# manasakani/Accelerated-Kinetic-Monte-Carlo-simulations-of-atomistically-resolved-resistive-memory-arrays

Hardware: AMD Instinct MI355X
Metric: cg_iterations_per_sec (higher is better)
Workload: dtype f64; 1 GPU; synthetic_40nm_crossbar(tiles=8,fill=0.52,lines=2,seed=40,bwmin); rows=1597080, nnz=41834706, sites=1635480, partition=1-D block rows x 1, transport=single, solver=jacobi-pcg fixed 1411 iterations, halo_cols_rank0=0, neighbours_rank0=1

## Files before the change

accelerated-kinetic-monte-carlo-simulations-of-atomistically-resolved-resistive-memory-arrays_amd/csrc/kmcf_internal.hpp:

```cpp
#pragma once
#include <hip/hip_runtime.h>

#include <condition_variable>
#include <cstdarg>
#include <cstdint>
#include <cstdio>
#include <algorithm>
#include <cstdlib>
#include <mutex>
#include <type_traits>
#include <vector>

#include "kmcfield.h"
#include "kmcf_knobs.hpp"

void kmcf_set_error(const char *fmt, ...);

#define KMCF_HIP(call)                                                                       \
    do {                                                                                     \
        hipError_t e_ = (call);                                                              \
        if (e_ != hipSuccess) {                                                              \
            kmcf_set_error("%s:%d: %s -> %s", __FILE__, __LINE__, #call, hipGetErrorString(e_)); \
            return KMCF_ERR_HIP;                                                             \
        }                                                                                    \
// ... 188 lines not shown
    int spmv_grid_coded = 0;
    bool sell_ok = false;
    bool sell_dirty = true;
    std::vector<int> h_sell_cuts;
    bool sell_ident = false;
    bool sell_nt = false;
    int sell_lw = 10, sell_nq = 0;
    int n_sell_tiles = 0, sell_grid = 0;
    int64_t n_sell_wcols = 0, n_sell_entries = 0;
    int4 *d_sell_tile = nullptr;
    int2 *d_sell_wave = nullptr;
    int *d_sell_lrow = nullptr;
    int *d_sell_wcol = nullptr;
    unsigned short *d_sell = nullptr;
    int *d_sell_pos = nullptr;
    double *d_sellv = nullptr;
    bool sellv_dirty = true;
    int sellv_grid = 0;
    int n_chunks = 0;
    int *d_chunk_row = nullptr;
    std::vector<int> h_row_ptr;
};

struct kmcf_kstate {
    kmcf_comm *comm = nullptr;
    kmcf_matrix *K = nullptr;
    int N = 0, N_left = 0, N_right = 0, N_interface = 0;
    std::vector<int> h_row_ptr, h_col;
    std::vector<int> h_left_row_ptr, h_left_col, h_right_row_ptr, h_right_col;
    int *d_left_row_ptr = nullptr, *d_left_col = nullptr;
// ... 37 lines not shown
    KMCF_PATH_STREAM,
    KMCF_PATH_WINDOW,
    KMCF_PATH_WCODE,
    KMCF_PATH_SELL,
    KMCF_PATH_SELLV,
};

inline kmcf_spmv_path kmcf_interior_path(const kmcf_matrix *m)
{
    if (m->spmv_kind == 1) return KMCF_PATH_STREAM;
    if (m->spmv_kind != 2) return KMCF_PATH_VEC;
    if (m->coded && m->sell_ok && m->dict_n <= 3) return KMCF_PATH_SELL;
    if (!m->coded && m->sell_ok && m->sell_ident && m->sellv_grid > 0) return KMCF_PATH_SELLV;
    return m->coded ? KMCF_PATH_WCODE : KMCF_PATH_WINDOW;
}

inline int kmcf_interior_grid(const kmcf_matrix *m)
{
    switch (kmcf_interior_path(m)) {
        case KMCF_PATH_WCODE: return m->spmv_grid_coded;
        case KMCF_PATH_SELL: return m->sell_grid;
        case KMCF_PATH_SELLV: return m->sellv_grid;
        default: return m->spmv_grid;
    }
}

constexpr int KMCF_SELL_NQ[] = {8, 13, 16};

template <class F>
int kmcf_sell_instance(const kmcf_matrix *m, F &&f)
// ... 157 lines not shown
```

accelerated-kinetic-monte-carlo-simulations-of-atomistically-resolved-resistive-memory-arrays_amd/csrc/kmcf_knobs.hpp:

```cpp
#pragma once
#include <cstdlib>
#include <string>

enum kmcf_knob_id {
    KNOB_BRICK, KNOB_SPMV_KIND, KNOB_SPMV_CODED, KNOB_SPMV_SELL, KNOB_SPMV_SELLV, KNOB_SPMV_SELL_ROWS,
    KNOB_SPMV_SELL_SORT, KNOB_SPMV_NT, KNOB_SELL_NT, KNOB_LONG_ROW, KNOB_CB_SCALED, KNOB_SUB_DENSE, KNOB_SUB_STRIP,
    KNOB_EVENTS_PERSISTENT, KNOB_EVENTS_FULLSCAN, KNOB_EVENTS_PARTITIONED, KNOB_EV_TREL, KNOB_CG_VARIANT,
    KNOB_CG_RESIDENT, KNOB_CGR_TPB, KNOB_CGR_G1, KNOB_CGR_DELAY, KNOB_CGR_RDELAY, KNOB_CGR_ADAPT, KNOB_CGR_TIMEOUT_MS,
    KNOB_CGR_CLASSIC_TILES, KNOB_TRANSPORT, KNOB_P2P_WINDOW_MB, KNOB_P2P_TIMEOUT_MS, KNOB_P2P_DIRECT, KNOB_P2P_AR,
    KNOB_FORCE_COMM, KNOB_LOOPBACK_TIMEOUT_S, KNOB_DEVICE_SHARE, KNOB_ENTER_ALWAYS, KNOB_TRACE, KNOB_COUNT
};

enum kmcf_knob_scope { KNOB_SCOPE_NONE, KNOB_COMM, KNOB_CONNECT, KNOB_PROCESS };

enum kmcf_knob_kind { KNOB_SPEC_NONE, KNOB_ENUM, KNOB_INT, KNOB_F64, KNOB_FLAG };
struct kmcf_knob_spec {
    kmcf_knob_kind kind;
    const char *words;
    double lo, hi;
};
constexpr kmcf_knob_spec kv_enum(const char *words) { return {KNOB_ENUM, words, 0, 0}; }
constexpr kmcf_knob_spec kv_int(double lo, double hi) { return {KNOB_INT, nullptr, lo, hi}; }
constexpr kmcf_knob_spec kv_f64(double lo, double hi) { return {KNOB_F64, nullptr, lo, hi}; }
constexpr kmcf_knob_spec kv_flag() { return {KNOB_FLAG, "0|1", 0, 0}; }
// ... 12 lines not shown
    {KNOB_SPMV_KIND, "KMCF_SPMV_KIND", "window, else stream, else vec", "0 vec / 1 stream / 2 window", "SpMV kernel family (forced: the window plan is not judged)",
     KNOB_COMM, false, kv_enum("0|1|2")},
    {KNOB_SPMV_CODED, "KMCF_SPMV_CODED", "1", "0 / 1", "0: f64 values streamed even where they could be coded",
     KNOB_COMM, false, kv_enum("0|1")},
    {KNOB_SPMV_SELL, "KMCF_SPMV_SELL", "1", "0 / 1", "0: the coded window kernel instead of the row-per-lane kernel",
     KNOB_COMM, false, kv_enum("0|1")},
    {KNOB_SPMV_SELLV, "KMCF_SPMV_SELLV", "1", "0 / 1", "0: f64 matrices on the window kernel instead of the row-per-lane one",
     KNOB_COMM, false, kv_enum("0|1")},
    {KNOB_SPMV_SELL_ROWS, "KMCF_SPMV_SELL_ROWS", "by size: 64 … 256", "64 … 256 (multiples of 64)", "rows per row-per-lane tile",
     KNOB_COMM, false, kv_enum("64|128|192|256")},
    {KNOB_SPMV_SELL_SORT, "KMCF_SPMV_SELL_SORT", "1", "0 / 1", "0: the rows of a tile are not sorted into the internal row order",
     KNOB_COMM, false, kv_enum("0|1")},
    {KNOB_SPMV_NT, "KMCF_SPMV_NT", "matrices beyond the caches", "0 / 1", "nontemporal matrix loads in the f64-value SpMV kernels",
     KNOB_COMM, false, kv_enum("0|1")},
    {KNOB_SELL_NT, "KMCF_SELL_NT", "beyond the Infinity Cache", "0 / 1", "nontemporal loads of the coded entry stream",
     KNOB_COMM, false, kv_enum("0|1")},
    {KNOB_LONG_ROW, "KMCF_LONG_ROW", "384", "entries; <= 0: none", "rows longer than this go to the long-row kernel",
     KNOB_COMM, false, kv_int(-1000000000, 1000000000)},
    {KNOB_CB_SCALED, "KMCF_CB_SCALED", "0", "0 / 1", "1: the CB-edge solve in the literal scaled form (a group: one more halo exchange)",
     KNOB_COMM, true, kv_enum("0|1")},
    {KNOB_SUB_DENSE, "KMCF_SUB_DENSE", "dense from a quarter full", "0 bitmap / 1 dense / 2 jagged",
     "tunnel block as bitmap / dense symmetric tiles / jagged tiles (one rank); all ranks of a group must agree",
     KNOB_COMM, true, kv_enum("0|1|2")},
    {KNOB_SUB_STRIP, "KMCF_SUB_STRIP", "16", ">= 1", "tunnel-block tiles per strip",
     KNOB_COMM, true, kv_int(1, 1000000)},
    {KNOB_EVENTS_PERSISTENT, "KMCF_EVENTS_PERSISTENT", "1", "0 / 1", "0: three launches per event instead of one persistent block per batch",
     KNOB_COMM, true, kv_enum("0|1")},
    {KNOB_EVENTS_FULLSCAN, "KMCF_EVENTS_FULLSCAN", "unset", "set", "the reference-style zero-out pass over the event list",
     KNOB_COMM, false, kv_flag()},
    {KNOB_EVENTS_PARTITIONED, "KMCF_EVENTS_PARTITIONED", "unset", "set", "the reference's partitioned multi-rank event step instead of the replicated one",
// ... 78 lines not shown
```

accelerated-kinetic-monte-carlo-simulations-of-atomistically-resolved-resistive-memory-arrays_amd/csrc/kmcf_matrix.hip:

```cpp
#include <algorithm>
#include <cstring>

#include "kmcf_internal.hpp"

namespace {

template <typename T>
int dev_upload(T **d, const std::vector<T> &h)
{
    size_t bytes = std::max<size_t>(h.size(), 1) * sizeof(T);
    KMCF_HIP(hipMalloc(reinterpret_cast<void **>(d), bytes));
    if (!h.empty()) KMCF_HIP(hipMemcpy(*d, h.data(), h.size() * sizeof(T), hipMemcpyHostToDevice));
    return KMCF_OK;
}

template <typename T>
int dev_alloc(T **d, size_t n)
{
    KMCF_HIP(hipMalloc(reinterpret_cast<void **>(d), std::max<size_t>(n, 1) * sizeof(T)));
    KMCF_HIP(hipMemset(*d, 0, std::max<size_t>(n, 1) * sizeof(T)));
    return KMCF_OK;
}

}
// ... 413 lines not shown
    KMCF_CHECK(m && info, KMCF_ERR_ARG, "kmcf_matrix_info: null argument");
    info->matrix_size = m->matrix_size;
    info->rows_this_rank = m->n_loc;
    info->nnz = m->nnz;
    info->number_of_neighbours = m->number_of_neighbours;
    info->halo_cols = m->n_halo;
    info->send_rows = m->n_send;
    info->boundary_rows = m->n_boundary_rows;
    info->spmv_kind = m->spmv_kind;
    const kmcf_spmv_path path = kmcf_interior_path(m);
    const bool sell = path == KMCF_PATH_SELL || path == KMCF_PATH_SELLV;
    const bool window = path == KMCF_PATH_WINDOW || path == KMCF_PATH_WCODE;
    info->spmv_coded = path == KMCF_PATH_SELL ? 2 : path == KMCF_PATH_WCODE ? 1 : 0;
    info->spmv_tiles = sell ? m->n_sell_tiles : window ? m->n_tiles : 0;
    info->spmv_window_cols = sell ? m->n_sell_wcols : window ? m->n_wcols : 0;
    info->spmv_stream_entries = sell ? m->n_sell_entries : path == KMCF_PATH_WCODE ? (int64_t)m->h_row_ptr[m->n_short] : 0;
    return KMCF_OK;
}

extern "C" int kmcf_matrix_neighbour(const kmcf_matrix *m, int k, int *neighbour_rank, int *nnz_block,
                                     int *ncols, int *h_cols, int *nrows, int *h_rows)
{
    KMCF_CHECK(m && k >= 0 && k < m->number_of_neighbours, KMCF_ERR_ARG, "kmcf_matrix_neighbour: k=%d out of range", k);
    if (neighbour_rank) *neighbour_rank = m->neighbours[k];
    if (nnz_block) *nnz_block = m->nnz_per_neighbour[k];
    if (ncols) *ncols = (int)m->cols_per_neighbour[k].size();
    if (nrows) *nrows = (int)m->rows_per_neighbour[k].size();
    if (h_cols) memcpy(h_cols, m->cols_per_neighbour[k].data(), m->cols_per_neighbour[k].size() * sizeof(int));
    if (h_rows) memcpy(h_rows, m->rows_per_neighbour[k].data(), m->rows_per_neighbour[k].size() * sizeof(int));
    return KMCF_OK;
}
// ... 43 lines not shown
```

accelerated-kinetic-monte-carlo-simulations-of-atomistically-resolved-resistive-memory-arrays_amd/csrc/kmcf_spmv.hip:

```cpp
#include <algorithm>
#include <cstdio>
#include <cstdlib>
#include <cstring>

#include <climits>

#include "kmcf_p2p_dev.hpp"

namespace {

__device__ __forceinline__ double wave_sum_width(double v, int width)
{
#pragma unroll
    for (int off = 32; off >= 1; off >>= 1)
        if (off < width) v += __shfl_xor(v, off, 64);
    return v;
}

__device__ __forceinline__ double block_sum_256(double v, double *lds4)
{
    v = kmcf_wave_sum64(v);
    const int lane = threadIdx.x & 63, w = threadIdx.x >> 6;
    if (lane == 0) lds4[w] = v;
    __syncthreads();
// ... 266 lines not shown
    }
}

typedef unsigned int sell_pair __attribute__((ext_vector_type(2)));
#define KMCF_SELL_LD(p) stream_load<NT>(p)
#define KMCF_SELL_LD2(p) (*(p))

template <int WQ>
struct sell_regs {
    double xr[WQ];
    double xrow, xown, dg;
    int row, nq, wn;
    bool valid;
};

template <int NQ, int LW, int ND, bool DOT, bool SKIP_BOUNDARY, bool IDENT, bool NT = false>
__global__ __launch_bounds__(KMCF_BLOCK) void spmv_sell_kernel(
    int n_tiles, const int4 *__restrict__ tile4, const int2 *__restrict__ swave, const int *__restrict__ lrow,
    const int *__restrict__ wcol, const sell_pair *__restrict__ stream, const double *__restrict__ x, double *__restrict__ y,
    const unsigned char *__restrict__ is_boundary, double *__restrict__ part, const kmcf_scalars *__restrict__ S,
    int check_done, const double *__restrict__ dict, const double *__restrict__ diagv)
{
    constexpr int W = 1 << LW, WQ = W / KMCF_BLOCK - 1, BUF = ND * W;
    typedef sell_regs<WQ> regs_t;
    __shared__ double xs[2 * BUF];
    if (check_done && S->done) return;
    const int tid = threadIdx.x;
    const int lane = tid & 63;
    const int wv = __builtin_amdgcn_readfirstlane(tid >> 6);
    double dv[ND];
#pragma unroll
    for (int c = 0; c < ND; ++c) dv[c] = dict[c];
    const int xcd = blockIdx.x & 7, bi = blockIdx.x >> 3, nb8 = gridDim.x >> 3;
    const int Cx = (n_tiles + 7) >> 3;
    const int gmax = min(Cx, n_tiles - xcd * Cx);
    const int nt = gmax > bi ? (gmax - bi + nb8 - 1) / nb8 : 0;
    double dot = 0.0;
    if (nt > 0) {
// ... 18 lines not shown
            } else {
                t.valid = lr >= 0;
                t.row = d.x + (t.valid ? lr : 0);
            }
            t.xrow = x[t.row];
            t.xown = IDENT ? t.xrow : x[d.x + min(tid, d.y - 1)];
            t.dg = KMCF_SELL_LD2(diagv + t.row);
            if (SKIP_BOUNDARY) t.valid = t.valid && is_boundary[t.row] == 0;
            t.nq = sw.y;
            t.wn = d.w;
        };
        int4 d1 = tile4[KMCF_TILE_OF(1)], d2 = tile4[KMCF_TILE_OF(2)];
        int2 s1 = swave[KMCF_TILE_OF(1) * 4 + wv], s2 = swave[KMCF_TILE_OF(2) * 4 + wv];
        int wca[WQ], wcb[WQ], lra = 0, lrb = 0;
        regs_t ta, tb;
        sell_pair pk[NQ];
        {
            const int4 d0 = tile4[c_first];
            const int2 s0 = swave[c_first * 4 + wv];
            load_b(c_first, d0, wca, lra);
            load_b_pinned(KMCF_TILE_OF(1), d1, wcb, lrb);
            __builtin_amdgcn_sched_barrier(0);
            load_c(d0, s0, wca, lra, ta);
            const sell_pair *sp = stream + s0.x + lane;
            const int last = max(s0.y - 1, 0);
#pragma unroll
            for (int q = 0; q < NQ; ++q) pk[q] = KMCF_SELL_LD(sp + min(q, last) * 64);
        }
        auto body = [&](int k, regs_t &cur, regs_t &nxt, double *xb, int (&wu)[WQ], int &lu, int (&wl)[WQ], int &ll) {
#pragma unroll
            for (int c = 0; c < ND; ++c) xb[c * W + tid] = dv[c] * cur.xown;
#pragma unroll
            for (int q = 0; q < WQ; ++q) {
                const int slot = q * KMCF_BLOCK + tid;
                const double v = slot < cur.wn ? cur.xr[q] : 0.0;
#pragma unroll
                for (int c = 0; c < ND; ++c) xb[c * W + KMCF_BLOCK + slot] = dv[c] * v;
            }
            load_b(KMCF_TILE_OF(k + 2), d2, wl, ll);
            __builtin_amdgcn_sched_barrier(0);
            load_c(d1, s1, wu, lu, nxt);
            const sell_pair *spn = stream + s1.x + lane;
            const int lastn = max(s1.y - 1, 0);
            d1 = d2; s1 = s2;
            d2 = tile4[KMCF_TILE_OF(k + 3)];
            s2 = swave[KMCF_TILE_OF(k + 3) * 4 + wv];
            __syncthreads();
            const char *base = reinterpret_cast<const char *>(xb);
            double s = 0.0;
#pragma unroll
            for (int q = 0; q < NQ; ++q) {
                if (q < cur.nq) {
                    const sell_pair e = pk[q];
                    const double a0 = *reinterpret_cast<const double *>(base + (e.x & 0xffffu));
                    const double a1 = *reinterpret_cast<const double *>(base + (e.x >> 16));
                    const double a2 = *reinterpret_cast<const double *>(base + (e.y & 0xffffu));
                    const double a3 = *reinterpret_cast<const double *>(base + (e.y >> 16));
                    s += a0; s += a1; s += a2; s += a3;
                }
                pk[q] = KMCF_SELL_LD(spn + min(q, lastn) * 64);
            }
            if (cur.valid) {
                s += cur.dg * cur.xrow;
                y[cur.row] = s;
                if (DOT) dot += cur.xrow * s;
            }
        };
        int k = 0;
        for (; k + 1 < nt; k += 2) {
            body(k, ta, tb, xs, wcb, lrb, wca, lra);
            body(k + 1, tb, ta, xs + BUF, wca, lra, wcb, lrb);
        }
        if (k < nt) body(k, ta, tb, xs, wcb, lrb, wca, lra);
// ... 373 lines not shown
    with_bools([&](auto dot, auto skip) {
        run_or_query(spmv_wcode_kernel<WIN_U, WIN_WQ, dot, skip>, launch, &pc, grid, st, m->n_tiles, m->d_tile4, m->d_tbase, m->d_row_ptr,
                     m->d_wcol, m->d_idx16, m->d_p, m->d_Ap, isb, part, m->d_S, chk, m->d_dict, m->d_diagv);
    }, with_dot, skipb);
    return pc;
}

int sell_dispatch(kmcf_matrix *m, bool launch, bool with_dot, bool skip_if_done)
{
    constexpr int LW = 10;
    hipStream_t st = m->comm->stream;
    const int chk = skip_if_done ? 1 : 0, grid = launch ? kmcf_interior_grid(m) : 0;
    const bool skipb = (m->n_halo > 0);
    const unsigned char *isb = skipb ? m->d_is_boundary : nullptr;
    double *part = with_dot ? m->d_part_a : nullptr;
    const sell_pair *stream = reinterpret_cast<const sell_pair *>(m->d_sell);
    int pc = 0;
    kmcf_sell_instance(m, [&](auto nq, auto nd) {
        with_bools([&](auto dot, auto skip, auto ident) {
            auto run = [&](auto kernel) {
                run_or_query(kernel, launch, &pc, grid, st, m->n_sell_tiles, m->d_sell_tile, m->d_sell_wave, m->d_sell_lrow, m->d_sell_wcol,
                             stream, m->d_p, m->d_Ap, isb, part, m->d_S, chk, m->d_dict, m->d_diagv);
            };
            if constexpr (ident && !skip) {
                if (m->sell_nt && launch) return run(spmv_sell_kernel<nq, LW, nd, dot, false, true, true>);
            }
            run(spmv_sell_kernel<nq, LW, nd, dot, skip, ident>);
        }, with_dot, skipb, m->sell_ident);
        return 0;
    });
    return pc;
}

int sellv_dispatch(kmcf_matrix *m, bool launch, bool with_dot, bool skip_if_done)
{
    constexpr int LW = 10;
    hipStream_t st = m->comm->stream;
    const int chk = skip_if_done ? 1 : 0, grid = launch ? kmcf_interior_grid(m) : 0;
    const bool skipb = (m->n_halo > 0);
    const unsigned char *isb = skipb ? m->d_is_boundary : nullptr;
    double *part = with_dot ? m->d_part_a : nullptr;
    int pc = 0;
    with_bools([&](auto dot, auto skip) {
// ... 34 lines not shown
    const int lane = threadIdx.x % LPR;
    const unsigned int slot_part = (unsigned int)(((1 << lw) - 1) << 3);
    for (int r = blockIdx.x * RPB + threadIdx.x / LPR; r < n; r += gridDim.x * RPB) {
        const int b = row_ptr[r], e = row_ptr[r + 1], dp = diag_pos[r];
        const int len = e - b - (dp >= 0 ? 1 : 0);
        const int pos0 = sell_pos[r];
        for (int k = lane; k < len; k += LPR) {
            const int j = b + k + ((dp >= 0 && b + k >= dp) ? 1 : 0);
            const unsigned int code = (unsigned int)idx16[j] >> KMCF_SLOT_BITS;
            const int pos = pos0 + (k >> 2) * 256 + (k & 3);
            sell[pos] = (unsigned short)((sell[pos] & slot_part) | (code << (lw + 3)));
        }
    }
}

int sell_refresh(kmcf_matrix *m)
{
    if (!m->sell_dirty) return KMCF_OK;
    constexpr int LPR = 4;
    sell_refresh_kernel<LPR><<<grid_for(m->n_short, KMCF_BLOCK / LPR), KMCF_BLOCK, 0, m->comm->stream>>>(
        m->n_short, m->d_row_ptr, m->d_diag_pos, m->d_idx16, m->d_sell_pos, m->d_sell, m->sell_lw);
    KMCF_HIP(hipGetLastError());
    m->sell_dirty = false;
    return KMCF_OK;
}

int resident_grid(const kmcf_matrix *m, int per_cu, int n_tiles)
{
    int cus = 0;
    if (hipDeviceGetAttribute(&cus, hipDeviceAttributeMultiprocessorCount, m->comm->device) != hipSuccess) cus = 0;
    const int resident = per_cu * cus / kmcf_device_share();
    int g = grid_for(n_tiles, 1);
    if (resident >= 8 && g > resident) g = resident / 8 * 8;
    return g;
}

void launch_interior(kmcf_matrix *m, bool with_dot, bool skip_if_done)
{
    switch (kmcf_interior_path(m)) {
        case KMCF_PATH_SELL:
            if (sell_refresh(m) == KMCF_OK) sell_dispatch(m, true, with_dot, skip_if_done);
            break;
        case KMCF_PATH_SELLV:
            if (sellv_prepare(m) == KMCF_OK) sellv_dispatch(m, true, with_dot, skip_if_done);
            break;
        case KMCF_PATH_WCODE: wcode_dispatch(m, true, with_dot, skip_if_done); break;
        case KMCF_PATH_WINDOW: window_dispatch(m, true, with_dot, skip_if_done); break;
        case KMCF_PATH_STREAM: stream_dispatch(m, with_dot, skip_if_done); break;
        case KMCF_PATH_VEC: launch_vec_any(m, with_dot, skip_if_done, false); break;
    }
}

bool coding_allowed(const kmcf_comm *c) { return kmcf_opt_int(c, KNOB_SPMV_CODED, 1) != 0; }
bool sell_allowed(const kmcf_comm *c) { return kmcf_opt_int(c, KNOB_SPMV_SELL, 1) != 0; }

int plan_sell(kmcf_matrix *m, const std::vector<int> &col);
// ... 147 lines not shown
    const sell_params sp = sell_plan_params(m->comm, n);
    const int lw = sp.lw, W = 1 << lw, row_cap = sp.row_cap;
    int maxlen = 0;
    for (int i = 0; i < n; ++i) maxlen = std::max(maxlen, rp[i + 1] - rp[i] - (dpos[i] >= 0 ? 1 : 0));
    int nq = 0;
    for (int v : KMCF_SELL_NQ)
        if (4 * v >= maxlen) { nq = v; break; }
    if (nq == 0) return KMCF_OK;
    const unsigned short pad = (unsigned short)((W - 1) << 3);
    std::vector<int> slot((size_t)m->n_loc + m->n_halo, -1), uniq, touched, wcol, ord, pos((size_t)n, 0);
    std::vector<unsigned char> mark((size_t)m->n_loc + m->n_halo, 0);
    std::vector<int4> tiles;
    std::vector<int2> waves;
    std::vector<int> lrow;
    std::vector<unsigned short> st;
    int64_t real = 0;
    bool ident = true;
    auto len_of = [&](int i) { return rp[i + 1] - rp[i] - (dpos[i] >= 0 ? 1 : 0); };
    int r = 0;
    size_t next_cut = 0;
    const std::vector<int> &cuts = m->h_sell_cuts;
    while (r < n) {
        while (next_cut < cuts.size() && cuts[next_cut] <= r) ++next_cut;
        const bool given = next_cut < cuts.size() && cuts[next_cut] <= n && cuts[next_cut] - r <= row_cap;
        const int e_max = given ? cuts[next_cut] : n;
        const int e = sell_cut_tile(r, e_max, row_cap, given ? INT_MAX : sp.ecap, [](int i) { return i; },
                                    [&](int i, auto f) {
                                        for (int j = rp[i]; j < rp[i + 1]; ++j)
                                            if (j != dpos[i]) f(col[j]);
                                    },
// ... 13 lines not shown
        std::sort(uniq.begin(), uniq.end());
        for (size_t q = 0; q < uniq.size(); ++q) slot[uniq[q]] = KMCF_BLOCK + (int)q;
        const int nr = e - r;
        sell_lane_order(nr, [&](int a) { return len_of(r + a); }, ord);
        for (int i = 0; i < nr; ++i) ident = ident && ord[i] == i;
        tiles.push_back(make_int4(r, nr, (int)wcol.size(), (int)uniq.size()));
        for (int t = 0; t < KMCF_BLOCK; ++t) lrow.push_back(t < nr ? ord[t] : -1);
        for (int w = 0; w < KMCF_BLOCK / 64; ++w) {
            const int t0 = 64 * w;
            int wlen = 0;
            for (int t = t0; t < std::min(t0 + 64, nr); ++t) wlen = std::max(wlen, len_of(r + ord[t]));
            const int wq = (wlen + 3) / 4;
            const size_t base = st.size() / 4;
            waves.push_back(make_int2((int)base, wq));
            st.resize(st.size() + (size_t)wq * 256, pad);
            for (int t = t0; t < std::min(t0 + 64, nr); ++t) {
                const int row = r + ord[t];
                pos[row] = (int)((base + (t - t0)) * 4);
                int k = 0;
                for (int j = rp[row]; j < rp[row + 1]; ++j) {
                    if (j == dpos[row]) continue;
                    st[(size_t)pos[row] + (size_t)(k >> 2) * 256 + (k & 3)] = (unsigned short)(slot[col[j]] << 3);
                    ++k;
                }
                real += k;
            }
        }
        for (int cj : touched) slot[cj] = -1;
        wcol.insert(wcol.end(), uniq.begin(), uniq.end());
        r = e;
    }
    if (st.size() / 4 > (size_t)0x7fffff00 || (double)st.size() > 1.5 * (double)real + 4096.0 * tiles.size()) return KMCF_OK;
    const int nt = (int)tiles.size();
    const bool trace = kmcf_trace(m->comm);
    if (trace)
        fprintf(stderr, "kmcf row-per-lane plan: %d tiles of <= %d rows%s, %.1f rows, %.1f window columns per tile, %lld entries + %.1f %% padding, %d steps\n",
                nt, row_cap, ident ? " (sorted in place)" : "", double(n) / nt, double(wcol.size()) / nt, (long long)real, 100.0 * (double(st.size()) / double(std::max<int64_t>(real, 1)) - 1.0), nq);
    if (trace) {
        std::vector<long long> hist(20, 0), rows(20, 0);
        for (const int2 &w : waves) ++hist[std::min(w.y, 19)];
        for (int i = 0; i < n; ++i) ++rows[std::min((len_of(i) + 3) / 4, 19)];
        long long runs = 0, lines = 0;
        for (const int4 &t : tiles)
            for (int q = 0; q < t.w; ++q) {
                if (q == 0 || wcol[t.z + q] != wcol[t.z + q - 1] + 1) ++runs;
                if (q == 0 || wcol[t.z + q] / 8 != wcol[t.z + q - 1] / 8) ++lines;
            }
        fprintf(stderr, "  window: %.1f runs of consecutive columns, %.1f 64-byte lines of x per tile\n", double(runs) / nt, double(lines) / nt);
        fprintf(stderr, "  steps: waves / rows ");
// ... 5 lines not shown
    m->n_sell_wcols = (int64_t)wcol.size();
    st.resize(st.size() + 128 * 4, pad);
    wcol.push_back(0);
    KMCF_HIP(hipMalloc(reinterpret_cast<void **>(&m->d_sell_tile), tiles.size() * sizeof(int4)));
    KMCF_HIP(hipMalloc(reinterpret_cast<void **>(&m->d_sell_wave), waves.size() * sizeof(int2)));
    KMCF_HIP(hipMalloc(reinterpret_cast<void **>(&m->d_sell_lrow), lrow.size() * sizeof(int)));
    KMCF_HIP(hipMalloc(reinterpret_cast<void **>(&m->d_sell_wcol), wcol.size() * sizeof(int)));
    KMCF_HIP(hipMalloc(reinterpret_cast<void **>(&m->d_sell), st.size() * sizeof(unsigned short)));
    KMCF_HIP(hipMalloc(reinterpret_cast<void **>(&m->d_sell_pos), (size_t)n * sizeof(int)));
    KMCF_HIP(hipMemcpy(m->d_sell_tile, tiles.data(), tiles.size() * sizeof(int4), hipMemcpyHostToDevice));
    KMCF_HIP(hipMemcpy(m->d_sell_wave, waves.data(), waves.size() * sizeof(int2), hipMemcpyHostToDevice));
    KMCF_HIP(hipMemcpy(m->d_sell_lrow, lrow.data(), lrow.size() * sizeof(int), hipMemcpyHostToDevice));
    KMCF_HIP(hipMemcpy(m->d_sell_wcol, wcol.data(), wcol.size() * sizeof(int), hipMemcpyHostToDevice));
    KMCF_HIP(hipMemcpy(m->d_sell, st.data(), st.size() * sizeof(unsigned short), hipMemcpyHostToDevice));
    KMCF_HIP(hipMemcpy(m->d_sell_pos, pos.data(), (size_t)n * sizeof(int), hipMemcpyHostToDevice));
    m->n_sell_tiles = nt;
    m->sell_lw = lw;
    m->sell_nq = nq;
    m->sell_dirty = true;
    m->sell_ident = ident;
    m->sell_ok = true;
    m->sell_grid = 0;
    m->sell_nt = 2.0 * (double)st.size() + 4.0 * (double)wcol.size() + 28.0 * (double)n > 300e6;
    m->sell_nt = kmcf_opt_int(m->comm, KNOB_SELL_NT, m->sell_nt) != 0;
    return KMCF_OK;
}

template <int LPR>
__global__ __launch_bounds__(KMCF_BLOCK) void encode_values_kernel(int n, const int *__restrict__ row_ptr,
                                                                   const int *__restrict__ diag_pos,
                                                                   const double *__restrict__ val,
                                                                   const double *__restrict__ dict, int nd,
                                                                   unsigned short *__restrict__ idx16,
                                                                   double *__restrict__ diagv, int *__restrict__ fail)
{
    __shared__ double sdict[64];
    if (threadIdx.x < 64) sdict[threadIdx.x] = dict[threadIdx.x];
    __syncthreads();
// ... 83 lines not shown
    for (int k = 0; k < 64; ++k) {
        const double v = k < nd ? h_dict[k] : 0.0;
        if (memcmp(&m->h_dict[k], &v, sizeof(v)) != 0) { same = false; m->h_dict[k] = v; }
    }
    if (!same || !m->dict_uploaded) {
        KMCF_HIP(hipMemcpyAsync(m->d_dict, m->h_dict, sizeof(m->h_dict), hipMemcpyHostToDevice, m->comm->stream));
        m->dict_uploaded = true;
    }
    if (m->spmv_grid_coded <= 0) m->spmv_grid_coded = resident_grid(m, wcode_dispatch(m, false, true, false), m->n_tiles);
    if (m->sell_ok && (m->sell_grid <= 0 || (m->dict_n <= 2) != (nd <= 2))) {
        m->dict_n = nd;
        m->sell_grid = resident_grid(m, sell_dispatch(m, false, true, false), m->n_sell_tiles);
        if (kmcf_trace(m->comm)) fprintf(stderr, "kmcf row-per-lane kernel: grid %d for %d tiles\n", m->sell_grid, m->n_sell_tiles);
    }
    m->dict_n = nd;
    m->sell_dirty = true;
    m->coded = true;
    return KMCF_OK;
}

int kmcf_matrix_encode_values(kmcf_matrix *m, const double *h_dict, int nd)
{
    kmcf_values_changed(m);
    if (!coding_enabled(m) || m->n_short == 0) return KMCF_OK;
    hipStream_t st = m->comm->stream;
    KMCF_TRY(kmcf_matrix_set_dictionary(m, h_dict, nd));
    m->coded = false;
    KMCF_HIP(hipMemsetAsync(m->d_code_fail, 0, sizeof(int), st));
    constexpr int LPR = 16;
    encode_values_kernel<LPR><<<grid_for(m->n_short, KMCF_BLOCK / LPR), KMCF_BLOCK, 0, st>>>(
        m->n_short, m->d_row_ptr, m->d_diag_pos, m->d_val, m->d_dict, nd, m->d_idx16, m->d_diagv, m->d_code_fail);
// ... 89 lines not shown
    }
    if (m->n_long_items > 0) {
        hipStream_t st = m->comm->stream;
        const int chk = skip_if_done ? 1 : 0;
        double *part = m->d_part_a + 2 * KMCF_MAX_PARTIALS;
        with_bools([&](auto dot) {
            spmv_long_kernel<dot><<<m->n_long_items, KMCF_BLOCK, 0, st>>>(m->n_long_items, m->d_long_items, m->d_col, m->d_val, m->d_p,
                                                                         m->d_Ap, m->d_long_part, m->d_long_ctr, part, m->d_S, chk);
        }, with_dot);
        KMCF_HIP(hipGetLastError());
    }
    if (m->sub) KMCF_TRY(kmcf_subop_finish(m, with_dot, skip_if_done));
    return KMCF_OK;
}

int kmcf_sell_ready(kmcf_matrix *m) { return sell_refresh(m); }

kmcf_part4 kmcf_spmv_partials(const kmcf_matrix *m)
{
    kmcf_part4 q;
    q.p[0] = m->d_part_a;                           q.n[0] = kmcf_interior_grid(m);
    q.p[1] = m->d_part_a + KMCF_MAX_PARTIALS;       q.n[1] = m->n_halo > 0 ? m->spmv_grid_b : 0;
    q.p[2] = m->d_part_a + 2 * KMCF_MAX_PARTIALS;   q.n[2] = m->n_long_items > 0 ? 1 : 0;
    q.p[3] = m->d_part_a + 3 * KMCF_MAX_PARTIALS;   q.n[3] = m->sub ? m->sub->grid : 0;
    return q;
}

extern "C" int kmcf_matrix_sum_plan(const kmcf_matrix *m, kmcf_sum_plan_t *plan, int *h_tile_first, int *h_tile_rows,
                                    int *h_row_ptr, int *h_col, double *h_val)
{
    KMCF_CHECK(m, KMCF_ERR_ARG, "kmcf_matrix_sum_plan: null matrix");
// ... 142 lines not shown
        const int nr = e - i;
        sell_lane_order(nr, [&](int a) { return len[i + a]; }, ord);
        tmp.resize((size_t)nr);
        for (int t = 0; t < nr; ++t) tmp[t] = perm[i + ord[t]];
        std::copy(tmp.begin(), tmp.end(), perm.begin() + i);
        for (int t = 0; t < nr; ++t) tmp[t] = len[i + ord[t]];
        std::copy(tmp.begin(), tmp.end(), len.begin() + i);
        i = e;
    }
}

void kmcf_spmv_plan_free(kmcf_matrix *m)
{
    void *ptrs[] = {m->d_chunk_row, m->d_tile, m->d_tile4, m->d_tbase, m->d_wcol, m->d_idx16, m->d_dict, m->d_diagv,
                    m->d_diag_pos, m->d_code_fail, m->d_sell_tile, m->d_sell_wave, m->d_sell_lrow, m->d_sell_wcol,
                    m->d_sell, m->d_sell_pos, m->d_sellv};
    for (void *p : ptrs)
        if (p) hipFree(p);
    m->d_chunk_row = nullptr; m->d_tile = nullptr; m->d_tile4 = nullptr; m->d_tbase = nullptr; m->d_wcol = nullptr;
    m->d_idx16 = nullptr; m->d_dict = nullptr; m->d_diagv = nullptr; m->d_diag_pos = nullptr; m->d_code_fail = nullptr;
    m->d_sell_tile = nullptr; m->d_sell_wave = nullptr; m->d_sell_lrow = nullptr; m->d_sell_wcol = nullptr;
    m->d_sell = nullptr; m->d_sell_pos = nullptr; m->d_sellv = nullptr;
    m->n_chunks = 0; m->n_tiles = 0; m->n_sell_tiles = 0; m->sellv_grid = 0;
    m->sell_ok = false; m->dict_uploaded = false;
    kmcf_values_changed(m);
}

extern "C" int kmcf_spmv_replan(kmcf_matrix *m)
{
    KMCF_CHECK(m && m->d_val, KMCF_ERR_ARG, "kmcf_spmv_replan: bad matrix");
    KMCF_TRY(kmcf_enter(m->comm));
    KMCF_HIP(hipStreamSynchronize(m->comm->stream));
    kmcf_spmv_plan_free(m);
    kmcf_cgr_free(m);
    KMCF_TRY(kmcf_spmv_plan(m));
    std::vector<double> v((size_t)m->nnz);
    KMCF_HIP(hipMemcpy(v.data(), m->d_val, v.size() * sizeof(double), hipMemcpyDeviceToHost));
// ... 47 lines not shown
```

Baseline: 20620 iterations/s.

## Pack coded SELL entry stream into five 12-bit fields per 8-byte word

After: 21250 iterations/s, median of 6. +3.1%, better.

```diff
diff --git a/accelerated-kinetic-monte-carlo-simulations-of-atomistically-resolved-resistive-memory-arrays_amd/csrc/kmcf_internal.hpp b/accelerated-kinetic-monte-carlo-simulations-of-atomistically-resolved-resistive-memory-arrays_amd/csrc/kmcf_internal.hpp
--- a/accelerated-kinetic-monte-carlo-simulations-of-atomistically-resolved-resistive-memory-arrays_amd/csrc/kmcf_internal.hpp
+++ b/accelerated-kinetic-monte-carlo-simulations-of-atomistically-resolved-resistive-memory-arrays_amd/csrc/kmcf_internal.hpp
@@ -226,6 +226,12 @@
     int *d_sell_wcol = nullptr;
     unsigned short *d_sell = nullptr;
     int *d_sell_pos = nullptr;
+    bool sell_pack = false;
+    bool sell12_dirty = true;
+    int64_t n_sell12_words = 0;
+    unsigned long long *d_sell12 = nullptr;
+    int2 *d_sell12_wave = nullptr;
+    int *d_sell12_pos = nullptr;
     double *d_sellv = nullptr;
     bool sellv_dirty = true;
     int sellv_grid = 0;
@@ -293,6 +299,8 @@
     if (!m->coded && m->sell_ok && m->sell_ident && m->sellv_grid > 0) return KMCF_PATH_SELLV;
     return m->coded ? KMCF_PATH_WCODE : KMCF_PATH_WINDOW;
 }
+
+inline bool kmcf_sell_packed(const kmcf_matrix *m) { return m->sell_pack && m->d_sell12 != nullptr; }
 
 inline int kmcf_interior_grid(const kmcf_matrix *m)
 {
diff --git a/accelerated-kinetic-monte-carlo-simulations-of-atomistically-resolved-resistive-memory-arrays_amd/csrc/kmcf_knobs.hpp b/accelerated-kinetic-monte-carlo-simulations-of-atomistically-resolved-resistive-memory-arrays_amd/csrc/kmcf_knobs.hpp
--- a/accelerated-kinetic-monte-carlo-simulations-of-atomistically-resolved-resistive-memory-arrays_amd/csrc/kmcf_knobs.hpp
+++ b/accelerated-kinetic-monte-carlo-simulations-of-atomistically-resolved-resistive-memory-arrays_amd/csrc/kmcf_knobs.hpp
@@ -4,7 +4,7 @@
 
 enum kmcf_knob_id {
     KNOB_BRICK, KNOB_SPMV_KIND, KNOB_SPMV_CODED, KNOB_SPMV_SELL, KNOB_SPMV_SELLV, KNOB_SPMV_SELL_ROWS,
-    KNOB_SPMV_SELL_SORT, KNOB_SPMV_NT, KNOB_SELL_NT, KNOB_LONG_ROW, KNOB_CB_SCALED, KNOB_SUB_DENSE, KNOB_SUB_STRIP,
+    KNOB_SPMV_SELL_SORT, KNOB_SPMV_NT, KNOB_SELL_NT, KNOB_SELL_PACK, KNOB_LONG_ROW, KNOB_CB_SCALED, KNOB_SUB_DENSE, KNOB_SUB_STRIP,
     KNOB_EVENTS_PERSISTENT, KNOB_EVENTS_FULLSCAN, KNOB_EVENTS_PARTITIONED, KNOB_EV_TREL, KNOB_CG_VARIANT,
     KNOB_CG_RESIDENT, KNOB_CGR_TPB, KNOB_CGR_G1, KNOB_CGR_DELAY, KNOB_CGR_RDELAY, KNOB_CGR_ADAPT, KNOB_CGR_TIMEOUT_MS,
     KNOB_CGR_CLASSIC_TILES, KNOB_TRANSPORT, KNOB_P2P_WINDOW_MB, KNOB_P2P_TIMEOUT_MS, KNOB_P2P_DIRECT, KNOB_P2P_AR,
@@ -50,6 +50,8 @@
     {KNOB_SPMV_NT, "KMCF_SPMV_NT", "matrices beyond the caches", "0 / 1", "nontemporal matrix loads in the f64-value SpMV kernels",
      KNOB_COMM, false, kv_enum("0|1")},
     {KNOB_SELL_NT, "KMCF_SELL_NT", "beyond the Infinity Cache", "0 / 1", "nontemporal loads of the coded entry stream",
+     KNOB_COMM, false, kv_enum("0|1")},
+    {KNOB_SELL_PACK, "KMCF_SELL_PACK", "1", "0 / 1", "0: the coded entry stream as 16-bit entries, four per 8-byte word, instead of five 12-bit fields",
      KNOB_COMM, false, kv_enum("0|1")},
     {KNOB_LONG_ROW, "KMCF_LONG_ROW", "384", "entries; <= 0: none", "rows longer than this go to the long-row kernel",
      KNOB_COMM, false, kv_int(-1000000000, 1000000000)},
diff --git a/accelerated-kinetic-monte-carlo-simulations-of-atomistically-resolved-resistive-memory-arrays_amd/csrc/kmcf_matrix.hip b/accelerated-kinetic-monte-carlo-simulations-of-atomistically-resolved-resistive-memory-arrays_amd/csrc/kmcf_matrix.hip
--- a/accelerated-kinetic-monte-carlo-simulations-of-atomistically-resolved-resistive-memory-arrays_amd/csrc/kmcf_matrix.hip
+++ b/accelerated-kinetic-monte-carlo-simulations-of-atomistically-resolved-resistive-memory-arrays_amd/csrc/kmcf_matrix.hip
@@ -451,7 +451,7 @@
     info->spmv_coded = path == KMCF_PATH_SELL ? 2 : path == KMCF_PATH_WCODE ? 1 : 0;
     info->spmv_tiles = sell ? m->n_sell_tiles : window ? m->n_tiles : 0;
     info->spmv_window_cols = sell ? m->n_sell_wcols : window ? m->n_wcols : 0;
-    info->spmv_stream_entries = sell ? m->n_sell_entries : path == KMCF_PATH_WCODE ? (int64_t)m->h_row_ptr[m->n_short] : 0;
+    info->spmv_stream_entries = path == KMCF_PATH_SELL && kmcf_sell_packed(m) ? 4 * m->n_sell12_words : sell ? m->n_sell_entries : path == KMCF_PATH_WCODE ? (int64_t)m->h_row_ptr[m->n_short] : 0;
     return KMCF_OK;
 }
 
diff --git a/accelerated-kinetic-monte-carlo-simulations-of-atomistically-resolved-resistive-memory-arrays_amd/csrc/kmcf_sell_pack.hpp b/accelerated-kinetic-monte-carlo-simulations-of-atomistically-resolved-resistive-memory-arrays_amd/csrc/kmcf_sell_pack.hpp
--- /dev/null
+++ b/accelerated-kinetic-monte-carlo-simulations-of-atomistically-resolved-resistive-memory-arrays_amd/csrc/kmcf_sell_pack.hpp
@@ -0,0 +1,62 @@
+#pragma once
+#include <cstdint>
+
+#if defined(__HIPCC__) || defined(__CUDACC__)
+#define KMCF_PACK_HD __host__ __device__ inline
+#else
+#define KMCF_PACK_HD inline
+#endif
+
+constexpr int KMCF_PACK_FIELDS = 5;
+constexpr int KMCF_PACK_BITS = 12;
+constexpr int KMCF_PACK_SLOT_BITS = 10;
+constexpr uint32_t KMCF_PACK_MASK = (1u << KMCF_PACK_BITS) - 1;
+
+KMCF_PACK_HD int kmcf_pack_steps(int len) { return (len + KMCF_PACK_FIELDS - 1) / KMCF_PACK_FIELDS; }
+
+KMCF_PACK_HD uint32_t kmcf_pack_field(uint32_t code, uint32_t slot) { return (code << KMCF_PACK_SLOT_BITS) | slot; }
+
+KMCF_PACK_HD uint32_t kmcf_pack_get(uint64_t w, int f) { return (uint32_t)(w >> (KMCF_PACK_BITS * f)) & KMCF_PACK_MASK; }
+
+KMCF_PACK_HD uint64_t kmcf_pack_put(uint64_t w, int f, uint32_t field)
+{
+    const int sh = KMCF_PACK_BITS * f;
+    return (w & ~((uint64_t)KMCF_PACK_MASK << sh)) | ((uint64_t)(field & KMCF_PACK_MASK) << sh);
+}
+
+KMCF_PACK_HD uint64_t kmcf_pack_put_code(uint64_t w, int f, uint32_t code)
+{
+    const int sh = KMCF_PACK_BITS * f + KMCF_PACK_SLOT_BITS;
+    constexpr uint64_t cmask = (1u << (KMCF_PACK_BITS - KMCF_PACK_SLOT_BITS)) - 1;
+    return (w & ~(cmask << sh)) | (((uint64_t)code & cmask) << sh);
+}
+
+KMCF_PACK_HD uint64_t kmcf_pack_fill(uint32_t field)
+{
+    uint64_t w = 0;
+    for (int f = 0; f < KMCF_PACK_FIELDS; ++f) w = kmcf_pack_put(w, f, field);
+    return w;
+}
+
+KMCF_PACK_HD void kmcf_pack_offsets(uint32_t lo, uint32_t hi, uint32_t (&off)[KMCF_PACK_FIELDS])
+{
+    off[0] = (lo & KMCF_PACK_MASK) << 3;
+    off[1] = ((lo >> 12) & KMCF_PACK_MASK) << 3;
+    off[2] = (((hi << 8) | (lo >> 24)) & KMCF_PACK_MASK) << 3;
+    off[3] = ((hi >> 4) & KMCF_PACK_MASK) << 3;
+    off[4] = ((hi >> 16) & KMCF_PACK_MASK) << 3;
+}
+
+KMCF_PACK_HD void kmcf_pack_row(const uint16_t *fields, int len, uint64_t *words, long stride)
+{
+    for (int k = 0; k < len; ++k) {
+        uint64_t &w = words[(long)(k / KMCF_PACK_FIELDS) * stride];
+        w = kmcf_pack_put(w, k % KMCF_PACK_FIELDS, fields[k]);
+    }
+}
+
+KMCF_PACK_HD void kmcf_unpack_row(const uint64_t *words, long stride, int len, uint16_t *fields)
+{
+    for (int k = 0; k < len; ++k)
+        fields[k] = (uint16_t)kmcf_pack_get(words[(long)(k / KMCF_PACK_FIELDS) * stride], k % KMCF_PACK_FIELDS);
+}
diff --git a/accelerated-kinetic-monte-carlo-simulations-of-atomistically-resolved-resistive-memory-arrays_amd/csrc/kmcf_spmv.hip b/accelerated-kinetic-monte-carlo-simulations-of-atomistically-resolved-resistive-memory-arrays_amd/csrc/kmcf_spmv.hip
--- a/accelerated-kinetic-monte-carlo-simulations-of-atomistically-resolved-resistive-memory-arrays_amd/csrc/kmcf_spmv.hip
+++ b/accelerated-kinetic-monte-carlo-simulations-of-atomistically-resolved-resistive-memory-arrays_amd/csrc/kmcf_spmv.hip
@@ -6,6 +6,7 @@
 #include <climits>
 
 #include "kmcf_p2p_dev.hpp"
+#include "kmcf_sell_pack.hpp"
 
 namespace {
 
@@ -304,7 +305,7 @@
     bool valid;
 };
 
-template <int NQ, int LW, int ND, bool DOT, bool SKIP_BOUNDARY, bool IDENT, bool NT = false>
+template <int NQ, int LW, int ND, bool DOT, bool SKIP_BOUNDARY, bool IDENT, bool NT = false, bool PACK = false>
 __global__ __launch_bounds__(KMCF_BLOCK) void spmv_sell_kernel(
     int n_tiles, const int4 *__restrict__ tile4, const int2 *__restrict__ swave, const int *__restrict__ lrow,
     const int *__restrict__ wcol, const sell_pair *__restrict__ stream, const double *__restrict__ x, double *__restrict__ y,
@@ -312,6 +313,8 @@
     int check_done, const double *__restrict__ dict, const double *__restrict__ diagv)
 {
     constexpr int W = 1 << LW, WQ = W / KMCF_BLOCK - 1, BUF = ND * W;
+    constexpr int NS = PACK ? (4 * NQ + KMCF_PACK_FIELDS - 1) / KMCF_PACK_FIELDS : NQ;
+    static_assert(!PACK || (LW == KMCF_PACK_SLOT_BITS && ND <= 4), "a packed field is 10 slot bits + 2 code bits");
     typedef sell_regs<WQ> regs_t;
     __shared__ double xs[2 * BUF];
     if (check_done && S->done) return;
@@ -360,7 +363,7 @@
         int2 s1 = swave[KMCF_TILE_OF(1) * 4 + wv], s2 = swave[KMCF_TILE_OF(2) * 4 + wv];
         int wca[WQ], wcb[WQ], lra = 0, lrb = 0;
         regs_t ta, tb;
-        sell_pair pk[NQ];
+        sell_pair pk[NS];
         {
             const int4 d0 = tile4[c_first];
             const int2 s0 = swave[c_first * 4 + wv];
@@ -371,7 +374,7 @@
             const sell_pair *sp = stream + s0.x + lane;
             const int last = max(s0.y - 1, 0);
 #pragma unroll
-            for (int q = 0; q < NQ; ++q) pk[q] = KMCF_SELL_LD(sp + min(q, last) * 64);
+            for (int q = 0; q < NS; ++q) pk[q] = KMCF_SELL_LD(sp + min(q, last) * 64);
         }
         auto body = [&](int k, regs_t &cur, regs_t &nxt, double *xb, int (&wu)[WQ], int &lu, int (&wl)[WQ], int &ll) {
 #pragma unroll
@@ -395,14 +398,24 @@
             const char *base = reinterpret_cast<const char *>(xb);
             double s = 0.0;
 #pragma unroll
-            for (int q = 0; q < NQ; ++q) {
+            for (int q = 0; q < NS; ++q) {
                 if (q < cur.nq) {
                     const sell_pair e = pk[q];
-                    const double a0 = *reinterpret_cast<const double *>(base + (e.x & 0xffffu));
-                    const double a1 = *reinterpret_cast<const double *>(base + (e.x >> 16));
-                    const double a2 = *reinterpret_cast<const double *>(base + (e.y & 0xffffu));
-                    const double a3 = *reinterpret_cast<const double *>(base + (e.y >> 16));
-                    s += a0; s += a1; s += a2; s += a3;
+                    if constexpr (PACK) {
+                        uint32_t off[KMCF_PACK_FIELDS];
+                        kmcf_pack_offsets(e.x, e.y, off);
+                        double a[KMCF_PACK_FIELDS];
+#pragma unroll
+                        for (int f = 0; f < KMCF_PACK_FIELDS; ++f) a[f] = *reinterpret_cast<const double *>(base + off[f]);
+#pragma unroll
+                        for (int f = 0; f < KMCF_PACK_FIELDS; ++f) s += a[f];
+                    } else {
+                        const double a0 = *reinterpret_cast<const double *>(base + (e.x & 0xffffu));
+                        const double a1 = *reinterpret_cast<const double *>(base + (e.x >> 16));
+                        const double a2 = *reinterpret_cast<const double *>(base + (e.y & 0xffffu));
+                        const double a3 = *reinterpret_cast<const double *>(base + (e.y >> 16));
+                        s += a0; s += a1; s += a2; s += a3;
+                    }
                 }
                 pk[q] = KMCF_SELL_LD(spn + min(q, lastn) * 64);
             }
@@ -806,19 +819,21 @@
     const bool skipb = (m->n_halo > 0);
     const unsigned char *isb = skipb ? m->d_is_boundary : nullptr;
     double *part = with_dot ? m->d_part_a : nullptr;
-    const sell_pair *stream = reinterpret_cast<const sell_pair *>(m->d_sell);
+    const bool packed = kmcf_sell_packed(m);
+    const sell_pair *stream = reinterpret_cast<const sell_pair *>(packed ? static_cast<const void *>(m->d_sell12) : m->d_sell);
+    const int2 *swave = packed ? m->d_sell12_wave : m->d_sell_wave;
     int pc = 0;
     kmcf_sell_instance(m, [&](auto nq, auto nd) {
-        with_bools([&](auto dot, auto skip, auto ident) {
+        with_bools([&](auto dot, auto skip, auto ident, auto pack) {
             auto run = [&](auto kernel) {
-                run_or_query(kernel, launch, &pc, grid, st, m->n_sell_tiles, m->d_sell_tile, m->d_sell_wave, m->d_sell_lrow, m->d_sell_wcol,
+                run_or_query(kernel, launch, &pc, grid, st, m->n_sell_tiles, m->d_sell_tile, swave, m->d_sell_lrow, m->d_sell_wcol,
                              stream, m->d_p, m->d_Ap, isb, part, m->d_S, chk, m->d_dict, m->d_diagv);
             };
             if constexpr (ident && !skip) {
-                if (m->sell_nt && launch) return run(spmv_sell_kernel<nq, LW, nd, dot, false, true, true>);
-            }
-            run(spmv_sell_kernel<nq, LW, nd, dot, skip, ident>);
-        }, with_dot, skipb, m->sell_ident);
+                if (m->sell_nt && launch) return run(spmv_sell_kernel<nq, LW, nd, dot, false, true, true, pack>);
+            }
+            run(spmv_sell_kernel<nq, LW, nd, dot, skip, ident, false, pack>);
+        }, with_dot, skipb, m->sell_ident, packed);
         return 0;
     });
     return pc;
@@ -883,8 +898,45 @@
     }
 }
 
-int sell_refresh(kmcf_matrix *m)
-{
+template <int LPR>
+__global__ __launch_bounds__(KMCF_BLOCK) void sell12_refresh_kernel(int n, const int *__restrict__ row_ptr,
+                                                                    const int *__restrict__ diag_pos,
+                                                                    const unsigned short *__restrict__ idx16,
+                                                                    const int *__restrict__ sell12_pos,
+                                                                    unsigned long long *__restrict__ sell12)
+{
+    constexpr int RPB = KMCF_BLOCK / LPR;
+    const int lane = threadIdx.x % LPR;
+    for (int r = blockIdx.x * RPB + threadIdx.x / LPR; r < n; r += gridDim.x * RPB) {
+        const int b = row_ptr[r], e = row_ptr[r + 1], dp = diag_pos[r];
+        const int len = e - b - (dp >= 0 ? 1 : 0);
+        unsigned long long *wp = sell12 + sell12_pos[r];
+        for (int q = lane; q * KMCF_PACK_FIELDS < len; q += LPR) {
+            uint64_t w = wp[(size_t)q * 64];
+#pragma unroll
+            for (int f = 0; f < KMCF_PACK_FIELDS; ++f) {
+                const int k = q * KMCF_PACK_FIELDS + f;
+                if (k < len) {
+                    const int j = b + k + ((dp >= 0 && b + k >= dp) ? 1 : 0);
+                    w = kmcf_pack_put_code(w, f, (unsigned int)idx16[j] >> KMCF_SLOT_BITS);
+                }
+            }
+            wp[(size_t)q * 64] = w;
+        }
+    }
+}
+
+int sell_refresh(kmcf_matrix *m, bool packed)
+{
+    if (packed) {
+        if (!m->sell12_dirty) return KMCF_OK;
+        constexpr int LPR12 = 4;
+        sell12_refresh_kernel<LPR12><<<grid_for(m->n_short, KMCF_BLOCK / LPR12), KMCF_BLOCK, 0, m->comm->stream>>>(
+            m->n_short, m->d_row_ptr, m->d_diag_pos, m->d_idx16, m->d_sell12_pos, m->d_sell12);
+        KMCF_HIP(hipGetLastError());
+        m->sell12_dirty = false;
+        return KMCF_OK;
+    }
     if (!m->sell_dirty) return KMCF_OK;
     constexpr int LPR = 4;
     sell_refresh_kernel<LPR><<<grid_for(m->n_short, KMCF_BLOCK / LPR), KMCF_BLOCK, 0, m->comm->stream>>>(
@@ -908,7 +960,7 @@
 {
     switch (kmcf_interior_path(m)) {
         case KMCF_PATH_SELL:
-            if (sell_refresh(m) == KMCF_OK) sell_dispatch(m, true, with_dot, skip_if_done);
+            if (sell_refresh(m, kmcf_sell_packed(m)) == KMCF_OK) sell_dispatch(m, true, with_dot, skip_if_done);
             break;
         case KMCF_PATH_SELLV:
             if (sellv_prepare(m) == KMCF_OK) sellv_dispatch(m, true, with_dot, skip_if_done);
@@ -1086,6 +1138,11 @@
     std::vector<int2> waves;
     std::vector<int> lrow;
     std::vector<unsigned short> st;
+    const bool want_pack = lw == KMCF_PACK_SLOT_BITS && kmcf_opt_int(m->comm, KNOB_SELL_PACK, 1) != 0;
+    const uint64_t pad12 = kmcf_pack_fill(kmcf_pack_field(0, (uint32_t)(W - 1)));
+    std::vector<uint64_t> st12;
+    std::vector<int2> waves12;
+    std::vector<int> pos12(want_pack ? (size_t)n : 0, 0);
     int64_t real = 0;
     bool ident = true;
     auto len_of = [&](int i) { return rp[i + 1] - rp[i] - (dpos[i] >= 0 ? 1 : 0); };
@@ -1129,13 +1186,23 @@
             const size_t base = st.size() / 4;
             waves.push_back(make_int2((int)base, wq));
             st.resize(st.size() + (size_t)wq * 256, pad);
+            const size_t base12 = st12.size();
+            if (want_pack) {
+                waves12.push_back(make_int2((int)base12, kmcf_pack_steps(wlen)));
+                st12.resize(base12 + (size_t)kmcf_pack_steps(wlen) * 64, pad12);
+            }
             for (int t = t0; t < std::min(t0 + 64, nr); ++t) {
                 const int row = r + ord[t];
                 pos[row] = (int)((base + (t - t0)) * 4);
+                if (want_pack) pos12[row] = (int)(base12 + (t - t0));
                 int k = 0;
                 for (int j = rp[row]; j < rp[row + 1]; ++j) {
                     if (j == dpos[row]) continue;
                     st[(size_t)pos[row] + (size_t)(k >> 2) * 256 + (k & 3)] = (unsigned short)(slot[col[j]] << 3);
+                    if (want_pack) {
+                        uint64_t &w12 = st12[(size_t)pos12[row] + (size_t)(k / KMCF_PACK_FIELDS) * 64];
+                        w12 = kmcf_pack_put(w12, k % KMCF_PACK_FIELDS, kmcf_pack_field(0, (uint32_t)slot[col[j]]));
+                    }
                     ++k;
                 }
                 real += k;
@@ -1148,6 +1215,12 @@
     if (st.size() / 4 > (size_t)0x7fffff00 || (double)st.size() > 1.5 * (double)real + 4096.0 * tiles.size()) return KMCF_OK;
     const int nt = (int)tiles.size();
     const bool trace = kmcf_trace(m->comm);
+    const bool pack = want_pack && st12.size() <= (size_t)0x7fffff00 &&
+                      (double)KMCF_PACK_FIELDS * (double)st12.size() <= 1.5 * (double)real + 5120.0 * tiles.size();
+    if (trace && pack)
+        fprintf(stderr, "kmcf row-per-lane plan: packed stream %lld words = %.1f MB (16-bit: %.1f MB), %lld entries + %.1f %% padding, %d steps\n",
+                (long long)st12.size(), 8e-6 * st12.size(), 2e-6 * st.size(), (long long)real,
+                100.0 * (double(KMCF_PACK_FIELDS) * double(st12.size()) / double(std::max<int64_t>(real, 1)) - 1.0), kmcf_pack_steps(4 * nq));
     if (trace)
         fprintf(stderr, "kmcf row-per-lane plan: %d tiles of <= %d rows%s, %.1f rows, %.1f window columns per tile, %lld entries + %.1f %% padding, %d steps\n",
                 nt, row_cap, ident ? " (sorted in place)" : "", double(n) / nt, double(wcol.size()) / nt, (long long)real, 100.0 * (double(st.size()) / double(std::max<int64_t>(real, 1)) - 1.0), nq);
@@ -1183,6 +1256,18 @@
     KMCF_HIP(hipMemcpy(m->d_sell_wcol, wcol.data(), wcol.size() * sizeof(int), hipMemcpyHostToDevice));
     KMCF_HIP(hipMemcpy(m->d_sell, st.data(), st.size() * sizeof(unsigned short), hipMemcpyHostToDevice));
     KMCF_HIP(hipMemcpy(m->d_sell_pos, pos.data(), (size_t)n * sizeof(int), hipMemcpyHostToDevice));
+    m->sell_pack = pack;
+    m->n_sell12_words = pack ? (int64_t)st12.size() : 0;
+    if (pack) {
+        st12.resize(st12.size() + 128, pad12);
+        KMCF_HIP(hipMalloc(reinterpret_cast<void **>(&m->d_sell12), st12.size() * sizeof(uint64_t)));
+        KMCF_HIP(hipMalloc(reinterpret_cast<void **>(&m->d_sell12_wave), waves12.size() * sizeof(int2)));
+        KMCF_HIP(hipMalloc(reinterpret_cast<void **>(&m->d_sell12_pos), (size_t)n * sizeof(int)));
+        KMCF_HIP(hipMemcpy(m->d_sell12, st12.data(), st12.size() * sizeof(uint64_t), hipMemcpyHostToDevice));
+        KMCF_HIP(hipMemcpy(m->d_sell12_wave, waves12.data(), waves12.size() * sizeof(int2), hipMemcpyHostToDevice));
+        KMCF_HIP(hipMemcpy(m->d_sell12_pos, pos12.data(), (size_t)n * sizeof(int), hipMemcpyHostToDevice));
+    }
+    m->sell12_dirty = true;
     m->n_sell_tiles = nt;
     m->sell_lw = lw;
     m->sell_nq = nq;
@@ -1190,7 +1275,8 @@
     m->sell_ident = ident;
     m->sell_ok = true;
     m->sell_grid = 0;
-    m->sell_nt = 2.0 * (double)st.size() + 4.0 * (double)wcol.size() + 28.0 * (double)n > 300e6;
+    const double stream_bytes = pack ? 8.0 * (double)m->n_sell12_words : 2.0 * (double)m->n_sell_entries;
+    m->sell_nt = stream_bytes + 4.0 * (double)m->n_sell_wcols + 28.0 * (double)n > 300e6;
     m->sell_nt = kmcf_opt_int(m->comm, KNOB_SELL_NT, m->sell_nt) != 0;
     return KMCF_OK;
 }
@@ -1304,7 +1390,7 @@
         if (kmcf_trace(m->comm)) fprintf(stderr, "kmcf row-per-lane kernel: grid %d for %d tiles\n", m->sell_grid, m->n_sell_tiles);
     }
     m->dict_n = nd;
-    m->sell_dirty = true;
+    m->sell_dirty = m->sell12_dirty = true;
     m->coded = true;
     return KMCF_OK;
 }
@@ -1424,7 +1510,7 @@
     return KMCF_OK;
 }
 
-int kmcf_sell_ready(kmcf_matrix *m) { return sell_refresh(m); }
+int kmcf_sell_ready(kmcf_matrix *m) { return sell_refresh(m, false); }
 
 kmcf_part4 kmcf_spmv_partials(const kmcf_matrix *m)
 {
@@ -1597,13 +1683,14 @@
 {
     void *ptrs[] = {m->d_chunk_row, m->d_tile, m->d_tile4, m->d_tbase, m->d_wcol, m->d_idx16, m->d_dict, m->d_diagv,
                     m->d_diag_pos, m->d_code_fail, m->d_sell_tile, m->d_sell_wave, m->d_sell_lrow, m->d_sell_wcol,
-                    m->d_sell, m->d_sell_pos, m->d_sellv};
+                    m->d_sell, m->d_sell_pos, m->d_sellv, m->d_sell12, m->d_sell12_wave, m->d_sell12_pos};
     for (void *p : ptrs)
         if (p) hipFree(p);
     m->d_chunk_row = nullptr; m->d_tile = nullptr; m->d_tile4 = nullptr; m->d_tbase = nullptr; m->d_wcol = nullptr;
     m->d_idx16 = nullptr; m->d_dict = nullptr; m->d_diagv = nullptr; m->d_diag_pos = nullptr; m->d_code_fail = nullptr;
     m->d_sell_tile = nullptr; m->d_sell_wave = nullptr; m->d_sell_lrow = nullptr; m->d_sell_wcol = nullptr;
     m->d_sell = nullptr; m->d_sell_pos = nullptr; m->d_sellv = nullptr;
+    m->d_sell12 = nullptr; m->d_sell12_wave = nullptr; m->d_sell12_pos = nullptr; m->sell_pack = false; m->n_sell12_words = 0;
     m->n_chunks = 0; m->n_tiles = 0; m->n_sell_tiles = 0; m->sellv_grid = 0;
     m->sell_ok = false; m->dict_uploaded = false;
     kmcf_values_changed(m);
```
